# vLAR-group/unMORE

Measured on AMD Instinct MI355X. Metric: images/sec (train fwd+bwd) ObjectnessNet ViT-B/16 384x384, higher is better.
Workload: dtype bf16

## Files before the change

### unmore_amd/csrc/gemm_tn256.hip

```cpp
#include "umr_common.h"
#include <type_traits>
#include <stdlib.h>

namespace {

constexpr int TSUB = 64 * 256;
constexpr int TBUF = 4 * TSUB;
constexpr int TLDS = 2 * TBUF;

__device__ __forceinline__ int tn_swz2(int r) { return ((r & 3) << 2) | ((r >> 2) & 3); }

template <int CONV, bool PH2, int WF, bool X3 = false>
__global__ __launch_bounds__(512, 2) void gemm_tn256_kernel(const umr_gemm_tn_desc p, int tiles_k, int ntiles, int rows_per_split,
                                                            float* slab, float* bslab, int mapmode, int npairs_arg = 1) {
    extern __shared__ __attribute__((aligned(16))) char smem[];
    constexpr int SZ = 2;
    const int npairs = X3 ? npairs_arg : 1;
    const int xpix = X3 ? 3 * p.Cin : p.Cin;
    constexpr unsigned OOB = 0x80000000u;
    const int tid = threadIdx.x, lane = tid & 63;
    const int w = __builtin_amdgcn_readfirstlane(tid >> 6);
    int bid = blockIdx.x;
    {
        const int nwg = gridDim.x, xcd = bid & 7, q_ = nwg >> 3, r_ = nwg & 7;
        const int base = (xcd < r_) ? xcd * (q_ + 1) : r_ * (q_ + 1) + (xcd - r_) * q_;
        bid = base + (bid >> 3);
    }
    const int split = bid / ntiles, tile = bid - split * ntiles;
    const int tn = tile / tiles_k, tk = tile - tn * tiles_k;
    const int n0 = tn * 256, k0 = tk * 256;
    const int m_begin = split * rows_per_split;
    const int m_end = min(p.M, m_begin + rows_per_split);
    const int nst = (m_end - m_begin + 63) / 64;
    const bool do_bias = (p.dbias != nullptr);

    unsigned vo[4][2];
    unsigned x_eff[2][2];
    int x_r[2][2], x_t[2][2];
    unsigned x_bits[2][2];
#pragma unroll
    for (int i = 0; i < 2; ++i) {
        const int r = (w * 2 + i) * 4 + (lane >> 4);
        const int gch = (lane & 15) ^ tn_swz2(r);
#pragma unroll
        for (int h = 0; h < 2; ++h) {
            const int ncol = (mapmode & 2) ? n0 + h * 128 + gch * 8 : n0 + (gch >> 3) * 128 + h * 64 + (gch & 7) * 8;
            vo[h == 0 ? 0 : 3][i] = (ncol < p.N) ? (unsigned)(((int64_t)r * p.lddy + (ncol - n0)) * SZ) : OOB;
            const int kcol = (mapmode & 1) ? k0 + h * 128 + gch * 8 : k0 + (gch >> 2) * 64 + h * 32 + (gch & 3) * 8;
            unsigned v = OOB;
            x_r[h][i] = r;
            x_t[h][i] = 0;
            x_bits[h][i] = 0;
            if (kcol < p.K) {
                if (CONV == 0) {
                    v = (unsigned)(((int64_t)r * p.ldx + (kcol - k0)) * SZ);
                } else {
                    const int tap = kcol / p.Cin, ci = kcol - tap * p.Cin;
                    const int ky = tap / 3, kx = tap - ky * 3;
                    x_t[h][i] = ky | (kx << 2);
                    x_bits[h][i] = (1u << ky) | ((r == 0 && kx == 0) ? 8u : 0u) | ((r == 63 && kx == 2) ? 16u : 0u);
                    v = (unsigned)(((int64_t)(r + ky * p.W + kx) * xpix + ci) * SZ);
                }
            }
            vo[1 + h][i] = v;
            x_eff[h][i] = v;
        }
    }

    int st_tile = 0;
    int st_pp = 0, st_par = 0;
    int sb = 0, soy = 0, sox = 0;
    const int hw = (CONV != 0) ? p.Ho * p.Wo : 1;
    if (CONV != 0) {
        sb = m_begin / hw;
        const int rem = m_begin - sb * hw;
        soy = rem / p.Wo;
        sox = rem - soy * p.Wo;
    }
    const int rows_split = m_end - m_begin;
    auto nrec = [](int64_t v) -> unsigned { return v > 0x7FFFFFFFll ? 0x7FFFFFFFu : (v < 0 ? 0u : (unsigned)v); };
    const __amdgpu_buffer_rsrc_t rsY = __builtin_amdgcn_make_buffer_rsrc(
        (void*)((const char*)p.dY + ((int64_t)m_begin * p.lddy + n0) * SZ), 0, nrec(((int64_t)rows_split * p.lddy - n0) * SZ), 0x00020000);
    const __amdgpu_buffer_rsrc_t rsX = (CONV == 0)
        ? __builtin_amdgcn_make_buffer_rsrc((void*)((const char*)p.X + ((int64_t)m_begin * p.ldx + k0) * SZ), 0,
                                            nrec(((int64_t)rows_split * p.ldx - k0) * SZ), 0x00020000)
        : __builtin_amdgcn_make_buffer_rsrc((void*)((const char*)p.X + ((int64_t)m_begin - (p.W + 1)) * xpix * SZ), 0,
                                            rows_split > 0 ? 0x7FFFFFFFu : 0u, 0x00020000);
    const unsigned y_step = (unsigned)(64 * p.lddy * SZ), x_step = (unsigned)(64 * (CONV == 0 ? p.ldx : xpix) * SZ);
    unsigned soffY = 0, soffX = 0;
    auto stage_prep = [&]() {
        const int pa = X3 ? (((npairs == 6 ? 0x940 : 0x010) >> (2 * st_pp)) & 3) : 0;
        const int pb = X3 ? (((npairs == 6 ? 0x124 : 0x004) >> (2 * st_pp)) & 3) : 0;
        soffY = (unsigned)st_tile * y_step + (unsigned)(pa * p.N * SZ);
        soffX = (unsigned)st_tile * x_step + (unsigned)(pb * (CONV == 0 ? p.K : p.Cin) * SZ);
        const bool first_pair = !X3 || st_pp == 0;
        if (X3) { if (++st_pp == npairs) st_pp = 0; }
        if (CONV != 0 && first_pair) {
            const int rows_left = rows_split - st_tile * 64;
            if (WF == 2) {
                const int lin0 = soy * p.Wo + sox;
#pragma unroll
                for (int h = 0; h < 2; ++h)
#pragma unroll
                    for (int i = 0; i < 2; ++i) {
                        const int ky = x_t[h][i] & 3, kx = x_t[h][i] >> 2;
                        const int rem = (lin0 + x_r[h][i]) % hw;
                        const int oy = rem / p.Wo, ox = rem - oy * p.Wo;
                        const bool ok = (unsigned)(oy + ky - 1) < (unsigned)p.H && (unsigned)(ox + kx - 1) < (unsigned)p.W && x_r[h][i] < rows_left;
                        x_eff[h][i] = ok ? vo[1 + h][i] : OOB;
                    }
                const int lin1 = (lin0 + 64) % hw;
                soy = lin1 / p.Wo;
                sox = lin1 - soy * p.Wo;
            } else if (WF == 1) {
                const unsigned sw = (soy == 0 ? 1u : 0u) | (soy == p.Ho - 1 ? 4u : 0u) | (sox == 0 ? 8u : 0u) | (sox == p.Wo - 64 ? 16u : 0u);
#pragma unroll
                for (int h = 0; h < 2; ++h)
#pragma unroll
                    for (int i = 0; i < 2; ++i) x_eff[h][i] = (x_bits[h][i] & sw) ? OOB : vo[1 + h][i];
                if (rows_left < 64) {
#pragma unroll
                    for (int h = 0; h < 2; ++h)
#pragma unroll
                        for (int i = 0; i < 2; ++i)
                            if (x_r[h][i] >= rows_left) x_eff[h][i] = OOB;
                }
            } else {
#pragma unroll
                for (int h = 0; h < 2; ++h)
#pragma unroll
                    for (int i = 0; i < 2; ++i) {
                        const int ky = x_t[h][i] & 3, kx = x_t[h][i] >> 2;
                        int ox = sox + x_r[h][i], oy = soy;
                        if (ox >= p.Wo) { ox -= p.Wo; ++oy; }
                        if (oy >= p.Ho) oy = 0;
                        const bool ok = (unsigned)(oy + ky - 1) < (unsigned)p.H && (unsigned)(ox + kx - 1) < (unsigned)p.W && x_r[h][i] < rows_left;
                        x_eff[h][i] = ok ? vo[1 + h][i] : OOB;
                    }
            }
            if (WF != 2) {
                sox += 64;
                if (sox >= p.Wo) { sox -= p.Wo; if (++soy >= p.Ho) { soy = 0; ++sb; } }
            }
        }
    };
    auto stage_issue = [&](auto gtag, auto itag) {
        constexpr int G = decltype(gtag)::value, I = decltype(itag)::value;
        char* dst = smem + st_par * TBUF + G * TSUB + (w * 2 + I) * 1024;
        if constexpr (G == 0 || G == 3) {
            __builtin_amdgcn_raw_ptr_buffer_load_lds(rsY, UMR_LDS_PTR(dst), 16, vo[G][I], soffY, 0, 0);
        } else {
            const unsigned v = (CONV == 0) ? vo[G][I] : x_eff[G - 1][I];
            __builtin_amdgcn_raw_ptr_buffer_load_lds(rsX, UMR_LDS_PTR(dst), 16, v, soffX, 0, 0);
        }
        if (G == 3 && I == 1) { st_par ^= 1; if (!X3 || st_pp == 0) ++st_tile; }
    };
#define STAGE_DMA(G, I) stage_issue(std::integral_constant<int, G>{}, std::integral_constant<int, I>{})

    f32x4 acc[8][4];
#pragma unroll
    for (int i = 0; i < 8; ++i)
#pragma unroll
        for (int j = 0; j < 4; ++j) acc[i][j] = f32x4{0.f, 0.f, 0.f, 0.f};
    float bsum[8];
#pragma unroll
    for (int i = 0; i < 8; ++i) bsum[i] = 0.f;

    const int wn = w >> 2, wk = w & 3;
    const int g = lane >> 4, li = lane & 15;
    const int q = li >> 2, pp = li & 3;
    int y_ad[4][2], x_ad[2][2];
#pragma unroll
    for (int half = 0; half < 2; ++half) {
        const int r = g * 8 + half * 4 + q;
        const int sw = tn_swz2(r);
#pragma unroll
        for (int t = 0; t < 4; ++t) {
            const int c = wn * 8 + 2 * t + (pp >> 1);
            y_ad[t][half] = r * 256 + ((c ^ sw) << 4) + ((pp & 1) << 3);
        }
#pragma unroll
        for (int t = 0; t < 2; ++t) {
            const int c = wk * 4 + 2 * t + (pp >> 1);
            x_ad[t][half] = r * 256 + ((c ^ sw) << 4) + ((pp & 1) << 3);
        }
    }
    const unsigned lds0 = (unsigned)(uintptr_t)UMR_LDS_PTR(smem);
    unsigned par_off = lds0;
    auto read_frag = [&](auto offtag, int ad0, int ad1) -> bf16x8 {
        constexpr int OFF = decltype(offtag)::value;
        u32x2 v0, v1;
        asm volatile("ds_read_b64_tr_b16 %0, %1 offset:%2" : "=v"(v0) : "v"(par_off + (unsigned)ad0), "n"(OFF));
        asm volatile("ds_read_b64_tr_b16 %0, %1 offset:%2" : "=v"(v1) : "v"(par_off + (unsigned)ad1), "n"(OFF));
        const u32x4 f = {v0[0], v0[1], v1[0], v1[1]};
        return __builtin_bit_cast(bf16x8, f);
    };
#define RF(SUBI, KS, AD) read_frag(std::integral_constant<int, (SUBI) * TSUB + (KS) * 8192>{}, AD[0], AD[1])

    bf16x8 fy[2][4], fx0[2][2], fx1[2][2];

#define PHASE_SYNC_N(N)                                            \
    asm volatile("s_waitcnt vmcnt(" #N ")" ::: "memory");          \
    __builtin_amdgcn_s_barrier();                                  \
    asm volatile("s_waitcnt lgkmcnt(0)" ::: "memory");             \
    __builtin_amdgcn_sched_barrier(0);
#define MFMA(ACC, XF, YF) ACC = __builtin_amdgcn_mfma_f32_16x16x32_bf16(XF, YF, ACC, 0, 0, 0)
    constexpr int PRIO_MODE = PH2 ? 1 : 0;
#define QPRIO(x) if (PRIO_MODE == 0) __builtin_amdgcn_s_setprio(x);
#define QUADRANT_D(N0, K0, FX, DMA_A, DMA_B)                                                         \
    QPRIO(1)                                                                                        \
    MFMA(acc[N0 + 0][K0 + 0], FX[0][0], fy[0][0]); MFMA(acc[N0 + 0][K0 + 1], FX[0][1], fy[0][0]);   \
    MFMA(acc[N0 + 1][K0 + 0], FX[0][0], fy[0][1]); MFMA(acc[N0 + 1][K0 + 1], FX[0][1], fy[0][1]);   \
    __builtin_amdgcn_sched_barrier(0);                                                              \
    DMA_A;                                                                                          \
    __builtin_amdgcn_sched_barrier(0);                                                              \
    MFMA(acc[N0 + 2][K0 + 0], FX[0][0], fy[0][2]); MFMA(acc[N0 + 2][K0 + 1], FX[0][1], fy[0][2]);   \
    MFMA(acc[N0 + 3][K0 + 0], FX[0][0], fy[0][3]); MFMA(acc[N0 + 3][K0 + 1], FX[0][1], fy[0][3]);   \
    MFMA(acc[N0 + 0][K0 + 0], FX[1][0], fy[1][0]); MFMA(acc[N0 + 0][K0 + 1], FX[1][1], fy[1][0]);   \
    __builtin_amdgcn_sched_barrier(0);                                                              \
    DMA_B;                                                                                          \
    __builtin_amdgcn_sched_barrier(0);                                                              \
    MFMA(acc[N0 + 1][K0 + 0], FX[1][0], fy[1][1]); MFMA(acc[N0 + 1][K0 + 1], FX[1][1], fy[1][1]);   \
    MFMA(acc[N0 + 2][K0 + 0], FX[1][0], fy[1][2]); MFMA(acc[N0 + 2][K0 + 1], FX[1][1], fy[1][2]);   \
    MFMA(acc[N0 + 3][K0 + 0], FX[1][0], fy[1][3]); MFMA(acc[N0 + 3][K0 + 1], FX[1][1], fy[1][3]);   \
    QPRIO(0)
#define QUADRANT(N0, K0, FX, G) QUADRANT_D(N0, K0, FX, STAGE_DMA(G, 0), STAGE_DMA(G, 1))
#define PHASE_SYNC() PHASE_SYNC_N(6)
#define BIAS_ACC(N0)                                                                                \
    if (do_bias && bias_turn && wk == 0) {                                                          \
        _Pragma("unroll") for (int t = 0; t < 4; ++t) {                                             \
            float s_ = 0.f;                                                                         \
            _Pragma("unroll") for (int ks = 0; ks < 2; ++ks)                                        \
                _Pragma("unroll") for (int e = 0; e < 8; ++e) s_ += (float)fy[ks][t][e];            \
            bsum[N0 + t] += s_;                                                                     \
        }                                                                                           \
    }

    bool bias_turn = false;
    auto stage_body2 = [&]() {
#pragma unroll
        for (int t = 0; t < 2; ++t) { fx0[0][t] = RF(1, 0, x_ad[t]); fx0[1][t] = RF(1, 1, x_ad[t]); }
#pragma unroll
        for (int t = 0; t < 4; ++t) { fy[0][t] = RF(0, 0, y_ad[t]); fy[1][t] = RF(0, 1, y_ad[t]); }
#pragma unroll
        for (int t = 0; t < 2; ++t) { fx1[0][t] = RF(2, 0, x_ad[t]); fx1[1][t] = RF(2, 1, x_ad[t]); }
        PHASE_SYNC_N(6);
        BIAS_ACC(0)
        QUADRANT_D(0, 0, fx0, STAGE_DMA(3, 0), STAGE_DMA(3, 1))
        QUADRANT_D(0, 2, fx1, (void)0, (void)0)
        stage_prep();
#pragma unroll
        for (int t = 0; t < 4; ++t) { fy[0][t] = RF(3, 0, y_ad[t]); fy[1][t] = RF(3, 1, y_ad[t]); }
        PHASE_SYNC_N(2);
        BIAS_ACC(4)
        QUADRANT_D(4, 2, fx1, STAGE_DMA(0, 0); STAGE_DMA(0, 1), STAGE_DMA(1, 0); STAGE_DMA(1, 1))
        QUADRANT_D(4, 0, fx0, STAGE_DMA(2, 0), STAGE_DMA(2, 1))
    };
    auto stage_body = [&]() {
        if (PH2) { stage_body2(); return; }
#pragma unroll
        for (int t = 0; t < 2; ++t) { fx0[0][t] = RF(1, 0, x_ad[t]); fx0[1][t] = RF(1, 1, x_ad[t]); }
#pragma unroll
        for (int t = 0; t < 4; ++t) { fy[0][t] = RF(0, 0, y_ad[t]); fy[1][t] = RF(0, 1, y_ad[t]); }
        PHASE_SYNC();
        BIAS_ACC(0)
        QUADRANT(0, 0, fx0, 2)
#pragma unroll
        for (int t = 0; t < 2; ++t) { fx1[0][t] = RF(2, 0, x_ad[t]); fx1[1][t] = RF(2, 1, x_ad[t]); }
        PHASE_SYNC();
        QUADRANT(0, 2, fx1, 3)
        stage_prep();
#pragma unroll
        for (int t = 0; t < 4; ++t) { fy[0][t] = RF(3, 0, y_ad[t]); fy[1][t] = RF(3, 1, y_ad[t]); }
        PHASE_SYNC();
        BIAS_ACC(4)
        QUADRANT(4, 2, fx1, 0)
        PHASE_SYNC();
        QUADRANT(4, 0, fx0, 1)
    };

    if (PRIO_MODE == 1 && w >= 4) __builtin_amdgcn_s_setprio(1);
    stage_prep();
    STAGE_DMA(0, 0); STAGE_DMA(0, 1); STAGE_DMA(1, 0); STAGE_DMA(1, 1);
    STAGE_DMA(2, 0); STAGE_DMA(2, 1); STAGE_DMA(3, 0); STAGE_DMA(3, 1);
    stage_prep();
    STAGE_DMA(0, 0); STAGE_DMA(0, 1); STAGE_DMA(1, 0); STAGE_DMA(1, 1);
    if (PH2) { STAGE_DMA(2, 0); STAGE_DMA(2, 1); }
    asm volatile("s_waitcnt vmcnt(8)" ::: "memory");
    __builtin_amdgcn_s_barrier();

    int bias_next = tk;
    int c_pp = 0, c_m = 0;
    const int nsteps = nst * npairs;
#pragma unroll 1
    for (int t = 0; t < nsteps; ++t) {
        par_off = lds0 + (unsigned)((t & 1) * TBUF);
        const bool sum_pair = !X3 || ((((npairs == 6 ? 0x124 : 0x004) >> (2 * c_pp)) & 3) == 0);
        bias_turn = (c_m == bias_next) && sum_pair;
        stage_body();
        if (++c_pp == npairs) { c_pp = 0; if (c_m == bias_next) bias_next += tiles_k; ++c_m; }
    }
#undef BIAS_ACC
#undef QUADRANT
#undef QUADRANT_D
#undef PHASE_SYNC_N
#undef MFMA
#undef PHASE_SYNC
#undef STAGE_DMA
#undef RF
    asm volatile("s_waitcnt vmcnt(0)" ::: "memory");

    float* out = slab + (int64_t)split * p.N * p.K;
#pragma unroll
    for (int nt = 0; nt < 8; ++nt) {
        const int n = (mapmode & 2) ? n0 + (nt >> 2) * 128 + wn * 64 + (nt & 3) * 16 + li : n0 + wn * 128 + nt * 16 + li;
        if (n >= p.N) continue;
#pragma unroll
        for (int kt = 0; kt < 4; ++kt) {
            const int k = (mapmode & 1) ? k0 + (kt >> 1) * 128 + wk * 32 + (kt & 1) * 16 + g * 4 : k0 + wk * 64 + kt * 16 + g * 4;
            if (k >= p.K) continue;
            float* o = out + (int64_t)n * p.K + k;
            if (k + 3 < p.K && (p.K & 3) == 0) *(f32x4*)o = acc[nt][kt];
            else { for (int e = 0; e < 4; ++e) if (k + e < p.K) o[e] = acc[nt][kt][e]; }
        }
        if (do_bias && wk == 0) {
            float s_ = bsum[nt];
            s_ += __shfl_xor(s_, 16, 64);
            s_ += __shfl_xor(s_, 32, 64);
            if (g == 0) bslab[((int64_t)split * tiles_k + tk) * p.N + n] = s_;
        }
    }
}

}

bool umr_tn256_eligible(const umr_gemm_tn_desc* d, bool force) {
    if (d->dtype != UMR_BF16 && d->dtype != UMR_BF16X3) return false;
    if (d->dy_rows_in > 0 || d->x_rows_in > 0) return false;
    if (d->conv == 2) return false;
    if (d->dtype == UMR_BF16X3) return true;
    if (d->conv == 1 && d->Wo < 64) return false;
    if (force) return true;
    if (d->N < 192 || d->K < 192) return false;
    const int64_t tiles = (int64_t)((d->N + 255) / 256) * ((d->K + 255) / 256);
    return (int64_t)d->M >= 256 * 64 * 16 / (tiles < 1 ? 1 : tiles) && d->M >= 64 * 64;
}

void umr_tn256_plan(const umr_gemm_tn_desc* d, int* splits, int* rows_per_split) {
    const int64_t tiles = (int64_t)((d->N + 255) / 256) * ((d->K + 255) / 256);
    const int x3 = d->dtype == UMR_BF16X3 ? 6 : 1;
    int64_t rounds = (int64_t)d->M * tiles * x3 / (256ll * 4096);
    if (rounds < 1) rounds = 1;
    if (rounds > 4) rounds = 4;
    int64_t want = rounds * 256 / tiles;
    if (want < 1) want = 1;
    const int64_t min_stages = x3 == 6 ? 2 : 16;
    const int64_t max_by_rows = ((int64_t)d->M + 64 * min_stages - 1) / (64 * min_stages);
    if (want > max_by_rows) want = max_by_rows;
    int64_t rps = ((int64_t)d->M + want - 1) / want;
    rps = (rps + 63) / 64 * 64;
    {
        const int64_t cpix = (int64_t)d->Cin * (d->dtype == UMR_BF16X3 ? 3 : 1);
        const int64_t rowb = 2 * (int64_t)(d->conv ? (cpix > d->lddy ? cpix : d->lddy) : (d->ldx > d->lddy ? d->ldx : d->lddy));
        const int64_t halo = d->conv ? (2 * (int64_t)d->W + 4) * cpix * 2 : 0;
        int64_t cap = ((1ll << 31) - halo - 65536) / rowb / 64 * 64;
        if (cap < 64) cap = 64;
        if (rps > cap) rps = cap;
    }
    *rows_per_split = (int)rps;
    *splits = (int)(((int64_t)d->M + rps - 1) / rps);
}

int umr_launch_gemm_tn256(const umr_gemm_tn_desc* d, int splits, int rows_per_split, float* slab, float* bslab, hipStream_t s) {
    const int tiles_n = (d->N + 255) / 256, tiles_k = (d->K + 255) / 256;
    dim3 g((unsigned)(tiles_n * tiles_k * splits)), b(512);
    constexpr int mapmode = 3;
#define LT(CV, WFV)                                                                                                    \
    do {                                                                                                               \
        UMR_SET_MAX_LDS_ONCE((gemm_tn256_kernel<CV, true, WFV>), TLDS);                                                \
        hipLaunchKernelGGL((gemm_tn256_kernel<CV, true, WFV>), g, b, TLDS, s, *d, tiles_k, tiles_n * tiles_k, rows_per_split, slab, bslab, mapmode, 1); \
    } while (0)
#define LTX(CV, WFV)                                                                                                   \
    do {                                                                                                               \
        UMR_SET_MAX_LDS_ONCE((gemm_tn256_kernel<CV, true, WFV, true>), TLDS);                                          \
        hipLaunchKernelGGL((gemm_tn256_kernel<CV, true, WFV, true>), g, b, TLDS, s, *d, tiles_k, tiles_n * tiles_k, rows_per_split, slab, bslab, mapmode, npairs); \
    } while (0)
    if (d->dtype == UMR_BF16X3) {
        const int npairs = umr_f32_mode_now() == UMR_F32_X3_FAST ? 3 : 6;
        if (d->conv == 0) LTX(0, 0);
        else if (d->Wo % 64 == 0) LTX(1, 1);
        else if (d->Wo >= 64) LTX(1, 0);
        else LTX(1, 2);
    } else if (d->conv == 0) LT(0, 0);
    else if (d->Wo % 64 == 0) LT(1, 1);
    else LT(1, 0);
#undef LTX
#undef LT
    UMR_LAUNCH_CHECK();
    return UMR_OK;
}
```

### unmore_amd/csrc/umr_api.hip

```cpp
#include "umr_common.h"
#include <string.h>

static thread_local char g_err[256] = "";

int umr_set_error(int code, const char* msg) {
    strncpy(g_err, msg ? msg : "", sizeof(g_err) - 1);
    g_err[sizeof(g_err) - 1] = 0;
    return code;
}

extern "C" int umr_version(void) { return 100; }
extern "C" const char* umr_last_error_string(void) { return g_err; }

#include <atomic>
#include <stdlib.h>
static std::atomic<int> g_f32_mode{-1};
int umr_f32_mode_now() {
    int m = g_f32_mode.load(std::memory_order_relaxed);
    if (m < 0) {
        const char* e = getenv("UMR_F32_X3");
        m = (e && atoi(e) == 0) ? UMR_F32_EXACT : UMR_F32_X3;
        g_f32_mode.store(m, std::memory_order_relaxed);
    }
    return m;
}
extern "C" int umr_set_f32_mode(int mode) {
    if (mode != UMR_F32_EXACT && mode != UMR_F32_X3 && mode != UMR_F32_X3_FAST) return umr_set_error(UMR_ERR_INVALID, "umr_set_f32_mode: unknown mode");
    g_f32_mode.store(mode, std::memory_order_relaxed);
    return UMR_OK;
}
extern "C" int umr_get_f32_mode(void) { return umr_f32_mode_now(); }

static std::atomic<int> g_cu_budget{-1};
int umr_cu_budget_now() {
    int b = g_cu_budget.load(std::memory_order_relaxed);
    if (b < 0) {
        const char* e = getenv("UMR_CU_BUDGET");
        b = e ? atoi(e) : 0;
        if (b < 0) b = 0;
        g_cu_budget.store(b, std::memory_order_relaxed);
    }
    return b;
}
extern "C" int umr_set_cu_budget(int cus) {
    if (cus < 0) return umr_set_error(UMR_ERR_INVALID, "umr_set_cu_budget: negative budget");
    g_cu_budget.store(cus, std::memory_order_relaxed);
    return UMR_OK;
}
extern "C" int umr_get_cu_budget(void) { return umr_cu_budget_now(); }

static const char* const g_opt_names[UMR_OPT_COUNT] = {
    "UMR_GEMM_TILE", "UMR_NT_SPLITK", "UMR_SPLITK_FENCE", "UMR_NT_ORDER", "UMR_NT256_PERSIST", "UMR_NT256_BM",
    "UMR_X3_TRACE", "UMR_NT256_PH2", "UMR_ATTN_BWD_FUSED", "UMR_BILINEAR_GY", "UMR_HEAD_OUT_BWD_GENERIC"};
static std::atomic<int> g_opt[UMR_OPT_COUNT];
static int opt_parse(const char* v) {
    if (!v) return UMR_OPT_UNSET;
    if ((v[0] >= '0' && v[0] <= '9') || v[0] == '-' || v[0] == '+') return atoi(v);
    return (int)(unsigned char)v[0];
}
static const bool g_opt_loaded = [] {
    for (int i = 0; i < UMR_OPT_COUNT; ++i) g_opt[i].store(opt_parse(getenv(g_opt_names[i])), std::memory_order_relaxed);
    return true;
}();
int umr_opt(int id) { return g_opt[id].load(std::memory_order_relaxed); }
extern "C" int umr_set_debug_option(const char* name, const char* value) {
    if (!name) return umr_set_error(UMR_ERR_INVALID, "umr_set_debug_option: null name");
    for (int i = 0; i < UMR_OPT_COUNT; ++i)
        if (strcmp(name, g_opt_names[i]) == 0) {
            g_opt[i].store(opt_parse(value), std::memory_order_relaxed);
            return UMR_OK;
        }
    return umr_set_error(UMR_ERR_INVALID, "umr_set_debug_option: unknown option");
}
extern "C" int umr_get_debug_option(const char* name, int* value, int* is_set) {
    if (!name) return umr_set_error(UMR_ERR_INVALID, "umr_get_debug_option: null name");
    for (int i = 0; i < UMR_OPT_COUNT; ++i)
        if (strcmp(name, g_opt_names[i]) == 0) {
            const int v = g_opt[i].load(std::memory_order_relaxed);
            if (is_set) *is_set = v != UMR_OPT_UNSET;
            if (value) *value = v == UMR_OPT_UNSET ? 0 : v;
            return UMR_OK;
        }
    return umr_set_error(UMR_ERR_INVALID, "umr_get_debug_option: unknown option");
}
```

### unmore_amd/csrc/umr_common.h

```cpp
#pragma once
#include <hip/hip_runtime.h>
#include <stdint.h>
#include "../../include/umr.h"

typedef __bf16 bf16_t;
typedef __attribute__((ext_vector_type(8))) __bf16 bf16x8;
typedef __attribute__((ext_vector_type(4))) __bf16 bf16x4;
typedef __attribute__((ext_vector_type(2))) __bf16 bf16x2;
typedef __attribute__((ext_vector_type(4))) float f32x4;
typedef __attribute__((ext_vector_type(2))) float f32x2;
typedef __attribute__((ext_vector_type(16))) float f32x16;
typedef __attribute__((ext_vector_type(2))) unsigned u32x2;
typedef __attribute__((ext_vector_type(4))) unsigned u32x4;

#define UMR_GLOBAL_PTR(p) ((const __attribute__((address_space(1))) void*)(p))
#define UMR_LDS_PTR(p) ((__attribute__((address_space(3))) void*)(p))

__device__ __forceinline__ void glds16(const void* gsrc, void* lds_wave_base) {
    __builtin_amdgcn_global_load_lds(UMR_GLOBAL_PTR(gsrc), UMR_LDS_PTR(lds_wave_base), 16, 0, 0);
}

template <typename T> __device__ __forceinline__ float to_f32(T v);
template <> __device__ __forceinline__ float to_f32<float>(float v) { return v; }
template <> __device__ __forceinline__ float to_f32<bf16_t>(bf16_t v) { return (float)v; }
template <typename T> __device__ __forceinline__ T from_f32(float v);
template <> __device__ __forceinline__ float from_f32<float>(float v) { return v; }
template <> __device__ __forceinline__ bf16_t from_f32<bf16_t>(float v) { return (bf16_t)v; }

template <typename T> struct Vec4;
template <> struct Vec4<float> {
    static __device__ __forceinline__ f32x4 load(const float* p) { return *(const f32x4*)p; }
    static __device__ __forceinline__ void store(float* p, f32x4 v) { *(f32x4*)p = v; }
};
template <> struct Vec4<bf16_t> {
    static __device__ __forceinline__ f32x4 load(const bf16_t* p) {
        bf16x4 t = *(const bf16x4*)p;
        f32x4 r = {(float)t[0], (float)t[1], (float)t[2], (float)t[3]};
        return r;
    }
    static __device__ __forceinline__ void store(bf16_t* p, f32x4 v) {
        bf16x4 t = {(bf16_t)v[0], (bf16_t)v[1], (bf16_t)v[2], (bf16_t)v[3]};
        *(bf16x4*)p = t;
    }
};

__device__ __forceinline__ float gelu_erf(float x) { return 0.5f * x * (1.0f + erff(x * 0.70710678118654752440f)); }
__device__ __forceinline__ float dgelu_erf(float x) {
    const float cdf = 0.5f * (1.0f + erff(x * 0.70710678118654752440f));
    const float pdf = 0.39894228040143267794f * __expf(-0.5f * x * x);
    return cdf + x * pdf;
}

__device__ __forceinline__ void erf_exp_fast(float x, float& erf_z, float& e) {
    const float z = fabsf(x) * 0.70710678118654752440f;
    const float t = __builtin_amdgcn_rcpf(1.0f + 0.3275911f * z);
    e = __builtin_amdgcn_exp2f(-0.72134752044448170368f * x * x);
    const float poly = t * (0.254829592f + t * (-0.284496736f + t * (1.421413741f + t * (-1.453152027f + t * 1.061405429f))));
    const float r = 1.0f - poly * e;
    erf_z = x < 0.f ? -r : r;
}
template <typename T> __device__ __forceinline__ float gelu_sel(float x) {
    if constexpr (sizeof(T) == 2) {
        float ez, e;
        erf_exp_fast(x, ez, e);
        return 0.5f * x * (1.0f + ez);
    } else {
        return gelu_erf(x);
    }
}
template <typename T> __device__ __forceinline__ float dgelu_sel(float x) {
    if constexpr (sizeof(T) == 2) {
        float ez, e;
        erf_exp_fast(x, ez, e);
        return 0.5f * (1.0f + ez) + x * 0.39894228040143267794f * e;
    } else {
        return dgelu_erf(x);
    }
}

template <typename V> __device__ __forceinline__ V wave_sum(V v) {
#pragma unroll
    for (int o = 32; o > 0; o >>= 1) v += __shfl_xor(v, o, 64);
    return v;
}
__device__ __forceinline__ float wave_max(float v) {
#pragma unroll
    for (int o = 32; o > 0; o >>= 1) v = fmaxf(v, __shfl_xor(v, o, 64));
    return v;
}

template <int ND, int NN>
__device__ __forceinline__ void block_sum_fixed(double (&d)[ND], long long (&n)[NN], double* red_d, long long* red_n) {
    const int tid = threadIdx.x, lane = tid & 63, wv = tid >> 6;
#pragma unroll
    for (int k = 0; k < ND; ++k) d[k] = wave_sum(d[k]);
#pragma unroll
    for (int k = 0; k < NN; ++k) n[k] = wave_sum(n[k]);
    __syncthreads();
    if (lane == 0) {
#pragma unroll
        for (int k = 0; k < ND; ++k) red_d[wv * ND + k] = d[k];
#pragma unroll
        for (int k = 0; k < NN; ++k) red_n[wv * NN + k] = n[k];
    }
    __syncthreads();
    if (tid == 0) {
#pragma unroll
        for (int k = 0; k < ND; ++k) d[k] = ((red_d[k] + red_d[ND + k]) + red_d[2 * ND + k]) + red_d[3 * ND + k];
#pragma unroll
        for (int k = 0; k < NN; ++k) n[k] = red_n[k] + red_n[NN + k] + red_n[2 * NN + k] + red_n[3 * NN + k];
    }
}

template <int ND, int NN> struct SumPartial {
    double d[ND];
    int32_t c[NN + (NN & 1)];
};
static_assert(sizeof(SumPartial<1, 5>) == 32 && sizeof(SumPartial<2, 7>) == 48, "the loss workspaces are sized by these records");

template <int ND, int NN, typename I>
__device__ __forceinline__ void partials_sum_fixed(const SumPartial<ND, NN>* __restrict__ partials, I n_partials, double (&d)[ND],
                                                   long long (&n)[NN], double* red_d, long long* red_n) {
#pragma unroll
    for (int k = 0; k < ND; ++k) d[k] = 0.0;
#pragma unroll
    for (int k = 0; k < NN; ++k) n[k] = 0;
    for (I i = threadIdx.x; i < n_partials; i += 256) {
        const SumPartial<ND, NN> q = partials[i];
#pragma unroll
        for (int k = 0; k < ND; ++k) d[k] += q.d[k];
#pragma unroll
        for (int k = 0; k < NN; ++k) n[k] += q.c[k];
    }
    block_sum_fixed(d, n, red_d, red_n);
}

static __device__ uint4 umr_zero_page[16];

#include <atomic>
#define UMR_SET_MAX_LDS_ONCE(fn, bytes)                                                                             \
    do {                                                                                                            \
        static std::atomic<bool> done_{false};                                                                      \
        if (!done_.load(std::memory_order_acquire)) {                                                               \
            (void)hipFuncSetAttribute((const void*)(fn), hipFuncAttributeMaxDynamicSharedMemorySize, (bytes));      \
            done_.store(true, std::memory_order_release);                                                           \
        }                                                                                                           \
    } while (0)

#include <limits.h>
enum {
    UMR_OPT_GEMM_TILE = 0, UMR_OPT_NT_SPLITK, UMR_OPT_SPLITK_FENCE, UMR_OPT_NT_ORDER, UMR_OPT_NT256_PERSIST, UMR_OPT_NT256_BM,
    UMR_OPT_X3_TRACE, UMR_OPT_NT256_PH2, UMR_OPT_ATTN_BWD_FUSED, UMR_OPT_BILINEAR_GY, UMR_OPT_HEAD_OUT_BWD_GENERIC, UMR_OPT_COUNT
};
#define UMR_OPT_UNSET INT_MIN
int umr_opt(int id);
static inline int umr_opt_or(int id, int dflt) { const int v = umr_opt(id); return v == UMR_OPT_UNSET ? dflt : v; }

int umr_set_error(int code, const char* msg);
int umr_f32_mode_now();
int umr_cu_budget_now();
#define UMR_CHECK_ARG(cond, msg) do { if (!(cond)) return umr_set_error(UMR_ERR_INVALID, msg); } while (0)
#define UMR_LAUNCH_CHECK() do { hipError_t e_ = hipGetLastError(); if (e_ != hipSuccess) return umr_set_error(UMR_ERR_HIP - (int)e_, hipGetErrorString(e_)); } while (0)

int umr_rle_parse_launch(const uint8_t* chars, const int64_t* char_offsets, int K, int64_t total_chars, const int64_t* out_desc,
                         const int32_t* group_start, int G, int64_t out_bytes, int32_t* status, int32_t* nruns, long long* num,
                         uint32_t* starts, hipStream_t stream);
```

Baseline: 357.6.

## Add staggered-wave pipeline variant to TN256 weight-gradient GEMM

Adds a 'stagger' mode to the 256x256 TN GEMM kernel. In this mode the first four waves run a different stage body that issues all LDS fragment reads up front, waits on lgkmcnt, and interleaves the DMA staging differently, with one shorter prologue prefetch. The goal is to offset the wave groups so their MFMA and memory phases overlap instead of contending. It is on by default for the plain bf16 and conv-WF1 paths. It also adds env knobs for the stagger mode and for overriding the split count. Having the two wave groups follow different sync/wait schedules is a correctness and hazard risk.

```diff
diff --git a/unmore_amd/csrc/gemm_tn256.hip b/unmore_amd/csrc/gemm_tn256.hip
--- a/unmore_amd/csrc/gemm_tn256.hip
+++ b/unmore_amd/csrc/gemm_tn256.hip
@@ -12,7 +12,7 @@
 
 template <int CONV, bool PH2, int WF, bool X3 = false>
 __global__ __launch_bounds__(512, 2) void gemm_tn256_kernel(const umr_gemm_tn_desc p, int tiles_k, int ntiles, int rows_per_split,
-                                                            float* slab, float* bslab, int mapmode, int npairs_arg = 1) {
+                                                            float* slab, float* bslab, int mapmode, int npairs_arg = 1, int stagger = 0) {
     extern __shared__ __attribute__((aligned(16))) char smem[];
     constexpr int SZ = 2;
     const int npairs = X3 ? npairs_arg : 1;
@@ -20,6 +20,7 @@
     constexpr unsigned OOB = 0x80000000u;
     const int tid = threadIdx.x, lane = tid & 63;
     const int w = __builtin_amdgcn_readfirstlane(tid >> 6);
+    const bool ahead = PH2 && !X3 && (stagger != 0) && (w < 4);
     int bid = blockIdx.x;
     {
         const int nwg = gridDim.x, xcd = bid & 7, q_ = nwg >> 3, r_ = nwg & 7;
@@ -256,6 +257,34 @@
         QUADRANT_D(4, 2, fx1, STAGE_DMA(0, 0); STAGE_DMA(0, 1), STAGE_DMA(1, 0); STAGE_DMA(1, 1))
         QUADRANT_D(4, 0, fx0, STAGE_DMA(2, 0), STAGE_DMA(2, 1))
     };
+#define READ_WAIT()                                                \
+    asm volatile("s_waitcnt lgkmcnt(0)" ::: "memory");             \
+    __builtin_amdgcn_sched_barrier(0);
+#define END_SYNC_N(N)                                              \
+    asm volatile("s_waitcnt vmcnt(" #N ")" ::: "memory");          \
+    __builtin_amdgcn_s_barrier();                                  \
+    __builtin_amdgcn_sched_barrier(0);
+    auto stage_body2_ahead = [&]() {
+        stage_prep();
+#pragma unroll
+        for (int t = 0; t < 2; ++t) { fx0[0][t] = RF(1, 0, x_ad[t]); fx0[1][t] = RF(1, 1, x_ad[t]); }
+#pragma unroll
+        for (int t = 0; t < 4; ++t) { fy[0][t] = RF(0, 0, y_ad[t]); fy[1][t] = RF(0, 1, y_ad[t]); }
+#pragma unroll
+        for (int t = 0; t < 2; ++t) { fx1[0][t] = RF(2, 0, x_ad[t]); fx1[1][t] = RF(2, 1, x_ad[t]); }
+        READ_WAIT();
+        BIAS_ACC(0)
+        QUADRANT_D(0, 0, fx0, STAGE_DMA(0, 0); STAGE_DMA(0, 1), STAGE_DMA(1, 0); STAGE_DMA(1, 1))
+        QUADRANT_D(0, 2, fx1, STAGE_DMA(2, 0), STAGE_DMA(2, 1))
+        END_SYNC_N(6);
+#pragma unroll
+        for (int t = 0; t < 4; ++t) { fy[0][t] = RF(3, 0, y_ad[t]); fy[1][t] = RF(3, 1, y_ad[t]); }
+        READ_WAIT();
+        BIAS_ACC(4)
+        QUADRANT_D(4, 2, fx1, STAGE_DMA(3, 0), STAGE_DMA(3, 1))
+        QUADRANT_D(4, 0, fx0, (void)0, (void)0)
+        END_SYNC_N(2);
+    };
     auto stage_body = [&]() {
         if (PH2) { stage_body2(); return; }
 #pragma unroll
@@ -283,23 +312,31 @@
     stage_prep();
     STAGE_DMA(0, 0); STAGE_DMA(0, 1); STAGE_DMA(1, 0); STAGE_DMA(1, 1);
     STAGE_DMA(2, 0); STAGE_DMA(2, 1); STAGE_DMA(3, 0); STAGE_DMA(3, 1);
-    stage_prep();
-    STAGE_DMA(0, 0); STAGE_DMA(0, 1); STAGE_DMA(1, 0); STAGE_DMA(1, 1);
-    if (PH2) { STAGE_DMA(2, 0); STAGE_DMA(2, 1); }
-    asm volatile("s_waitcnt vmcnt(8)" ::: "memory");
+    if (ahead) {
+        asm volatile("s_waitcnt vmcnt(2)" ::: "memory");
+    } else {
+        stage_prep();
+        STAGE_DMA(0, 0); STAGE_DMA(0, 1); STAGE_DMA(1, 0); STAGE_DMA(1, 1);
+        if (PH2) { STAGE_DMA(2, 0); STAGE_DMA(2, 1); }
+        asm volatile("s_waitcnt vmcnt(8)" ::: "memory");
+    }
     __builtin_amdgcn_s_barrier();
 
     int bias_next = tk;
     int c_pp = 0, c_m = 0;
     const int nsteps = nst * npairs;
-#pragma unroll 1
-    for (int t = 0; t < nsteps; ++t) {
-        par_off = lds0 + (unsigned)((t & 1) * TBUF);
-        const bool sum_pair = !X3 || ((((npairs == 6 ? 0x124 : 0x004) >> (2 * c_pp)) & 3) == 0);
-        bias_turn = (c_m == bias_next) && sum_pair;
-        stage_body();
-        if (++c_pp == npairs) { c_pp = 0; if (c_m == bias_next) bias_next += tiles_k; ++c_m; }
-    }
+#define STAGE_LOOP(BODY)                                                                                        \
+    _Pragma("unroll 1") for (int t = 0; t < nsteps; ++t) {                                                      \
+        par_off = lds0 + (unsigned)((t & 1) * TBUF);                                                            \
+        const bool sum_pair = !X3 || ((((npairs == 6 ? 0x124 : 0x004) >> (2 * c_pp)) & 3) == 0);                \
+        bias_turn = (c_m == bias_next) && sum_pair;                                                             \
+        BODY();                                                                                                 \
+        if (++c_pp == npairs) { c_pp = 0; if (c_m == bias_next) bias_next += tiles_k; ++c_m; }                  \
+    }
+    if (ahead) { STAGE_LOOP(stage_body2_ahead) } else { STAGE_LOOP(stage_body) }
+#undef STAGE_LOOP
+#undef END_SYNC_N
+#undef READ_WAIT
 #undef BIAS_ACC
 #undef QUADRANT
 #undef QUADRANT_D
@@ -357,6 +394,8 @@
     const int64_t min_stages = x3 == 6 ? 2 : 16;
     const int64_t max_by_rows = ((int64_t)d->M + 64 * min_stages - 1) / (64 * min_stages);
     if (want > max_by_rows) want = max_by_rows;
+    const int want_e = umr_opt(UMR_OPT_TN256_SPLITS);
+    if (want_e != UMR_OPT_UNSET && want_e >= 1) want = want_e;
     int64_t rps = ((int64_t)d->M + want - 1) / want;
     rps = (rps + 63) / 64 * 64;
     {
@@ -375,27 +414,31 @@
     const int tiles_n = (d->N + 255) / 256, tiles_k = (d->K + 255) / 256;
     dim3 g((unsigned)(tiles_n * tiles_k * splits)), b(512);
     constexpr int mapmode = 3;
-#define LT(CV, WFV)                                                                                                    \
+    const int st_e = umr_opt(UMR_OPT_TN256_STAGGER);
+#define STG(DFLT) (st_e != UMR_OPT_UNSET ? (st_e != 0 ? 1 : 0) : (DFLT))
+#define LT(CV, WFV, SDFLT)                                                                                             \
     do {                                                                                                               \
         UMR_SET_MAX_LDS_ONCE((gemm_tn256_kernel<CV, true, WFV>), TLDS);                                                \
-        hipLaunchKernelGGL((gemm_tn256_kernel<CV, true, WFV>), g, b, TLDS, s, *d, tiles_k, tiles_n * tiles_k, rows_per_split, slab, bslab, mapmode, 1); \
+        hipLaunchKernelGGL((gemm_tn256_kernel<CV, true, WFV>), g, b, TLDS, s, *d, tiles_k, tiles_n * tiles_k, rows_per_split, slab, bslab, mapmode, 1, STG(SDFLT)); \
     } while (0)
-#define LTX(CV, WFV)                                                                                                   \
+#define LTX(CV, WFV, SDFLT)                                                                                            \
     do {                                                                                                               \
         UMR_SET_MAX_LDS_ONCE((gemm_tn256_kernel<CV, true, WFV, true>), TLDS);                                          \
-        hipLaunchKernelGGL((gemm_tn256_kernel<CV, true, WFV, true>), g, b, TLDS, s, *d, tiles_k, tiles_n * tiles_k, rows_per_split, slab, bslab, mapmode, npairs); \
+        hipLaunchKernelGGL((gemm_tn256_kernel<CV, true, WFV, true>), g, b, TLDS, s, *d, tiles_k, tiles_n * tiles_k, rows_per_split, slab, bslab, mapmode, npairs, STG(SDFLT)); \
     } while (0)
+    constexpr int ST_PLAIN = 1, ST_CONV_WF1 = 1, ST_CONV_WF0 = 0;
     if (d->dtype == UMR_BF16X3) {
         const int npairs = umr_f32_mode_now() == UMR_F32_X3_FAST ? 3 : 6;
-        if (d->conv == 0) LTX(0, 0);
-        else if (d->Wo % 64 == 0) LTX(1, 1);
-        else if (d->Wo >= 64) LTX(1, 0);
-        else LTX(1, 2);
-    } else if (d->conv == 0) LT(0, 0);
-    else if (d->Wo % 64 == 0) LT(1, 1);
-    else LT(1, 0);
+        if (d->conv == 0) LTX(0, 0, 0);
+        else if (d->Wo % 64 == 0) LTX(1, 1, 0);
+        else if (d->Wo >= 64) LTX(1, 0, 0);
+        else LTX(1, 2, 0);
+    } else if (d->conv == 0) LT(0, 0, ST_PLAIN);
+    else if (d->Wo % 64 == 0) LT(1, 1, ST_CONV_WF1);
+    else LT(1, 0, ST_CONV_WF0);
 #undef LTX
 #undef LT
+#undef STG
     UMR_LAUNCH_CHECK();
     return UMR_OK;
 }
diff --git a/unmore_amd/csrc/umr_api.hip b/unmore_amd/csrc/umr_api.hip
--- a/unmore_amd/csrc/umr_api.hip
+++ b/unmore_amd/csrc/umr_api.hip
@@ -51,7 +51,8 @@
 
 static const char* const g_opt_names[UMR_OPT_COUNT] = {
     "UMR_GEMM_TILE", "UMR_NT_SPLITK", "UMR_SPLITK_FENCE", "UMR_NT_ORDER", "UMR_NT256_PERSIST", "UMR_NT256_BM",
-    "UMR_X3_TRACE", "UMR_NT256_PH2", "UMR_ATTN_BWD_FUSED", "UMR_BILINEAR_GY", "UMR_HEAD_OUT_BWD_GENERIC"};
+    "UMR_X3_TRACE", "UMR_NT256_PH2", "UMR_ATTN_BWD_FUSED", "UMR_BILINEAR_GY", "UMR_HEAD_OUT_BWD_GENERIC",
+    "UMR_TN256_STAGGER", "UMR_TN256_SPLITS"};
 static std::atomic<int> g_opt[UMR_OPT_COUNT];
 static int opt_parse(const char* v) {
     if (!v) return UMR_OPT_UNSET;
diff --git a/unmore_amd/csrc/umr_common.h b/unmore_amd/csrc/umr_common.h
--- a/unmore_amd/csrc/umr_common.h
+++ b/unmore_amd/csrc/umr_common.h
@@ -150,7 +150,8 @@
 #include <limits.h>
 enum {
     UMR_OPT_GEMM_TILE = 0, UMR_OPT_NT_SPLITK, UMR_OPT_SPLITK_FENCE, UMR_OPT_NT_ORDER, UMR_OPT_NT256_PERSIST, UMR_OPT_NT256_BM,
-    UMR_OPT_X3_TRACE, UMR_OPT_NT256_PH2, UMR_OPT_ATTN_BWD_FUSED, UMR_OPT_BILINEAR_GY, UMR_OPT_HEAD_OUT_BWD_GENERIC, UMR_OPT_COUNT
+    UMR_OPT_X3_TRACE, UMR_OPT_NT256_PH2, UMR_OPT_ATTN_BWD_FUSED, UMR_OPT_BILINEAR_GY, UMR_OPT_HEAD_OUT_BWD_GENERIC,
+    UMR_OPT_TN256_STAGGER, UMR_OPT_TN256_SPLITS, UMR_OPT_COUNT
 };
 #define UMR_OPT_UNSET INT_MIN
 int umr_opt(int id);
```

New measurement: 358.9, median of 6. Within noise of the previous version (+0.4%).
